# JohannesErnst/WeaSAL

Hardware: AMD Instinct MI355X
Metric: points/sec fwd+bwd KPFCNN on DALES spheres; achieved HBM GB/s on KPConv gather (higher is better)
Workload: dtype f32; 1 GPU; DALES_PseudoLabel KP-FCNN, in_radius=10m, 50k pts/sphere, batch=8, fp32, step = GPU pyramid + fwd + loss + bwd + SGD; contrast_loss term included (trainer_PseudoLabel.py:204-208); pyramid of the next batch overlapped on a second stream; parallelism=dp1, dist_world_size=1, allreduce_bytes=0

## Files before the change

### include/weasal_hip.h

```cpp
#ifndef WEASAL_HIP_H
#define WEASAL_HIP_H

#include <stdint.h>

#ifdef __cplusplus
extern "C" {
#endif

typedef enum {
    WS_OK = 0,
    WS_ERR_INVALID = 1,
    WS_ERR_UNSUPPORTED = 2,
    WS_ERR_HIP = 3,
    WS_ERR_EMPTY = 4,
    WS_ERR_CAPACITY = 5
} ws_status;

enum { WS_INFLUENCE_LINEAR = 0, WS_INFLUENCE_CONSTANT = 1, WS_INFLUENCE_GAUSSIAN = 2 };
enum { WS_AGGREGATION_SUM = 0, WS_AGGREGATION_CLOSEST = 1 };

const char* ws_last_error(void);
int64_t ws_launch_count(void);
const char* ws_version(void);
int ws_device_count(void);
// ... 87 lines not shown
int ws_radius_neighbors_fill(ws_neighbors_ws* ws, int32_t width,
                             int32_t* out_i32, int64_t* out_i64, void* stream);
int ws_radius_neighbors_search(ws_neighbors_ws* ws,
                               const float* queries, int64_t nq, const float* supports, int64_t ns,
                               const int32_t* h_q_lens, const int32_t* h_s_lens, int32_t nb,
                               float radius, int32_t width, int32_t* out_i32, int64_t* out_i64,
                               int32_t* h_max_count, void* stream);
int32_t ws_radius_neighbors_async_cap(int32_t width);
int ws_radius_neighbors_search_async(ws_neighbors_ws* ws,
                                     const float* queries, int64_t nq, const float* supports, int64_t ns,
                                     const int32_t* h_q_lens, const int32_t* h_s_lens, int32_t nb,
                                     float radius, int32_t width, int32_t* out_i32, int64_t* out_i64,
                                     int32_t* d_max_count, void* stream);
#define WS_NB_HIST_MAX 8192
int ws_radius_neighbors_histogram(ws_neighbors_ws* ws,
                                  const float* queries, int64_t nq, const float* supports, int64_t ns,
                                  const int32_t* h_q_lens, const int32_t* h_s_lens, int32_t nb,
                                  float radius, int64_t* hist, int32_t hist_n, void* stream);
int ws_radius_neighbors_nearest_async(ws_neighbors_ws* ws, const float* queries, int64_t nq, const float* supports,
                                      int64_t ns, const int32_t* h_q_lens, const int32_t* h_s_lens, int32_t nb,
                                      float radius, int32_t* out_i32, int64_t* out_i64, int32_t* d_any, void* stream);
int ws_radius_neighbors_order(const ws_neighbors_ws* ws, int32_t* out_order, void* stream);
const int32_t* ws_radius_neighbors_counts(const ws_neighbors_ws* ws);
int ws_radius_neighbors_fill_variant(int32_t cap, int32_t out_i32, int32_t beside, char* out, int32_t out_cap);
int ws_radius_neighbors_last_fills(const ws_neighbors_ws* ws, int32_t* caps, int32_t max, int32_t* n);

#define WS_NN_STATUS_NONFINITE_QUERY 1
int ws_nearest_neighbors(ws_neighbors_ws* ws,
                         const float* queries, int64_t nq, const float* supports, int64_t ns,
                         const int32_t* h_q_lens, const int32_t* h_s_lens, int32_t nb,
                         float cell, int32_t* out_i32, int64_t* out_i64, double* out_d2, int32_t* d_status, void* stream);

int ws_radius_neighbors_set_key_last(ws_neighbors_ws* ws, uint64_t* d_key_last);
int ws_radius_neighbors_reuse_grid(ws_neighbors_ws* ws, int32_t on);
int ws_radius_neighbors_grid_info(const ws_neighbors_ws* ws, int32_t* nb, int64_t* cells, int64_t* ns, int64_t* blob_bytes);
int ws_radius_neighbors_grid_export(const ws_neighbors_ws* ws, void* blob, void* stream);
int ws_kpconv_gather_bwd_x_grid(const float* s_pts, int64_t ns, const void* grid_blob, int32_t nb, int64_t cells,
                                const uint64_t* key_last, float radius, const float* dwf, int32_t ci,
                                const float* kernel_points, int32_t k, const float* deformed_kp, const float* modulations,
                                float extent, int32_t influence, int32_t aggregation, const int32_t* order, float* dx,
                                int32_t* overflow, void* stream);

int ws_kpconv_gather_bwd_x_gated(const float* q_pts, int64_t nq, const float* s_pts, int64_t ns,
                                 const int64_t* inds, int32_t h, const int32_t* t_offsets, const int32_t* t_pairs,
                                 const float* dwf, int32_t ci, const float* kernel_points, int32_t k,
                                 const float* deformed_kp, const float* modulations, float extent,
                                 int32_t influence, int32_t aggregation, const int32_t* order, const float* gate_y,
                                 float gate_slope, float* dx, void* stream);
int ws_kpconv_gather_bwd_x_packed(const float* q_pts, int64_t nq, const float* s_pts, int64_t ns,
                                  const int64_t* inds, int32_t h, const int32_t* t_offsets, const int32_t* t_pairs,
                                  const float* dwf, int32_t ci, const float* kernel_points, int32_t k,
                                  const float* deformed_kp, const float* modulations, float extent,
                                  int32_t influence, int32_t aggregation, const int32_t* order, const float* gate_y,
                                  float gate_slope, float* dx, void* stream);
int ws_kpconv_gather_bwd_x_packed_variant(int64_t nq, int64_t ns, int32_t h, int32_t ci, const void* dwf, const void* dx, int32_t deformed,
                                          int32_t modulated, int32_t influence, int32_t aggregation, int32_t rows_bf16, int32_t ordered,
                                          char* out, int32_t cap);
int ws_kpconv_gather_bwd_x_grid_gated(const float* s_pts, int64_t ns, const void* grid_blob, int32_t nb, int64_t cells,
                                      const uint64_t* key_last, float radius, const float* dwf, int32_t ci,
                                      const float* kernel_points, int32_t k, const float* deformed_kp, const float* modulations,
                                      float extent, int32_t influence, int32_t aggregation, const int32_t* order,
                                      const float* gate_y, float gate_slope, const int64_t* rows, int32_t rows_h, float* dx,
                                      int32_t* overflow, void* stream);

enum { WS_ORDER_REFERENCE = 0, WS_ORDER_FIRST_SEEN = 1 };
typedef struct ws_subsample_ws ws_subsample_ws;
// ... 441 lines not shown
```

### weasal_amd/csrc/neighbors.hip

```cpp
#include "neighbors_kernels.h"
#include "nearest_kernels.h"
#include "ws_dispatch.h"
#include <vector>
#include <algorithm>

namespace {

template <typename T>
struct DevBuf {
    T* p = nullptr;
    size_t cap = 0;
    int ensure(size_t n)
    {
        if (n <= cap) return WS_OK;
        if (p) (void)hipFree(p);
        p = nullptr; cap = 0;
        size_t want = n + n / 4 + 64;
        WS_HIP(hipMalloc((void**)&p, want * sizeof(T)));
        cap = want;
        return WS_OK;
    }
    void release() { if (p) (void)hipFree(p); p = nullptr; cap = 0; }
};

}

struct ws_neighbors_ws {
    DevBuf<CloudGrid> grids;
    DevBuf<float> bbox;
    DevBuf<int32_t> cell_of, cell_start, cursor, counts, scan_scratch, max_count;
    DevBuf<float4> sorted, sorted_alt;
    DevBuf<int32_t> order;
    bool self_query = false;
    const float* queries = nullptr;
    int64_t nq = 0, ns = 0;
    int nb = 0;
    float r2 = 0.f;
    int max_count_host = 0;
    int64_t cells = 0;
    int32_t* max_count_word = nullptr;
    unsigned long long* key_last = nullptr;
    bool reuse_next = false;
    const float* supports = nullptr;
    float radius = 0.f;
    bool auto_cell = false;
    std::vector<int32_t> s_lens;
    std::vector<int32_t> fills;
};

extern "C" {

int ws_neighbors_ws_create(ws_neighbors_ws** ws)
{
    WS_REQUIRE(ws, "NULL argument");
    *ws = new ws_neighbors_ws();
    return WS_OK;
}

void ws_neighbors_ws_destroy(ws_neighbors_ws* ws)
{
    if (!ws) return;
    ws->grids.release(); ws->bbox.release(); ws->cell_of.release(); ws->cell_start.release();
    ws->cursor.release(); ws->counts.release(); ws->scan_scratch.release(); ws->max_count.release();
    ws->sorted.release(); ws->sorted_alt.release(); ws->order.release();
    delete ws;
}

static int nb_prepare(ws_neighbors_ws* ws, const float* queries, int64_t nq, const float* supports, int64_t ns,
                      const int32_t* h_q_lens, const int32_t* h_s_lens, int32_t nb, float radius, hipStream_t st,
                      bool auto_cell = false)
{
    WS_REQUIRE(ws && h_q_lens && h_s_lens, "NULL argument");
    ws->fills.clear();
    WS_REQUIRE(nb >= 1 && nq >= 0 && ns >= 0, "bad sizes nb=%d nq=%lld ns=%lld", nb, (long long)nq, (long long)ns);
// ... 89 lines not shown
    return WS_OK;
}

static int nb_begin(ws_neighbors_ws* ws, const float* queries, int64_t nq, const float* supports, int64_t ns,
                    const int32_t* h_q_lens, const int32_t* h_s_lens, int32_t nb, float radius, hipStream_t st,
                    bool auto_cell = false)
{
    const int rc = nb_prepare(ws, queries, nq, supports, ns, h_q_lens, h_s_lens, nb, radius, st, auto_cell);
    if (rc && ws) ws->nq = 0;
    return rc;
}

int ws_radius_neighbors_plan(ws_neighbors_ws* ws, const float* queries, int64_t nq, const float* supports,
                             int64_t ns, const int32_t* h_q_lens, const int32_t* h_s_lens, int32_t nb,
                             float radius, int32_t* h_max_count, void* stream)
{
    WS_REQUIRE(h_max_count, "NULL argument");
    *h_max_count = 0;
    hipStream_t st = (hipStream_t)stream;
    int rc = nb_begin(ws, queries, nq, supports, ns, h_q_lens, h_s_lens, nb, radius, st);
    if (rc) return rc;
    nb_count_kernel<<<ws_grid(nq, 4), 256, 0, st>>>(queries, nq, ws->grids.p, nb, ws->cell_start.p, ws->sorted.p, ws->r2,
                                                    ws->self_query ? ws->order.p : nullptr, ws->counts.p, ws->max_count_word);
    WS_LAUNCH_CHECK();
    int32_t mc = 0;
    WS_HIP(hipMemcpyAsync(&mc, ws->max_count_word, sizeof(int32_t), hipMemcpyDeviceToHost, st));
    WS_HIP(hipStreamSynchronize(st));
    ws->max_count_host = mc;
    *h_max_count = mc;
    if (mc == 0) return ws_fail(WS_ERR_EMPTY, "Error");
    return WS_OK;
}

struct KeyLastGuard {
    ws_neighbors_ws* ws;
    ~KeyLastGuard() { if (ws) ws->key_last = nullptr; }
};

extern "C" int ws_nb_wide_caps = 1;
constexpr int NB_MAX_BLOCKS = 1024;

enum NbFillKernel { NB_FILL_NONE, NB_FILL_NEAREST, NB_FILL_128, NB_FILL_WIDE, NB_FILL_2048 };
struct NbFillPlan {
    NbFillKernel kernel;
    int slab;
    bool out_i32;
    int max_blocks;
};

static NbFillPlan nb_fill_plan(int cap, bool out_i32, bool beside)
{
    if (cap == 0) return {NB_FILL_NEAREST, 0, out_i32, 256 * 16};
    const int slab = cap <= 128 ? 128 : cap <= 576 ? 576 : cap <= 704 ? 704 : cap <= 1024 ? 1024 : cap <= 2048 ? 2048 : 0;
    const NbFillKernel kernel = !slab ? NB_FILL_NONE : slab == 128 ? NB_FILL_128 : slab == 2048 ? NB_FILL_2048 : NB_FILL_WIDE;
    return {kernel, slab, out_i32, beside ? NB_MAX_BLOCKS : 256 * 16};
}
static int nb_fill_unsupported(int cap)
{
    return ws_fail(WS_ERR_UNSUPPORTED, "max neighbour count %d exceeds the 2048-entry sort slab", cap);
}

static int nb_launch_fill(ws_neighbors_ws* ws, int cap, int32_t width, int32_t* out_i32, int64_t* out_i64,
                          bool with_counts, hipStream_t st, bool beside = false)
{
    const NbFillPlan p = nb_fill_plan(cap, out_i32 != nullptr, beside);
    if (p.kernel == NB_FILL_NONE) return nb_fill_unsupported(cap);
    const int grid = ws_grid(ws->nq, 4, p.max_blocks);
    const int32_t* qo = ws->self_query ? ws->order.p : nullptr;
    int32_t* cn = with_counts ? ws->counts.p : nullptr;
    int32_t* mx = with_counts ? ws->max_count_word : nullptr;
    unsigned long long* kl = ws->key_last;
    const bool called = dispatch([&](auto i32, auto sl) {
        using OT = std::conditional_t<i32.value != 0, int32_t, int64_t>;
        OT* out = i32.value ? (OT*)out_i32 : (OT*)out_i64;
        if constexpr (sl.value == 0)
            nb_nearest_kernel<OT><<<grid, 256, 0, st>>>(ws->queries, ws->nq, ws->grids.p, ws->nb, ws->cell_start.p, ws->sorted.p, ws->r2, ws->ns,
                                                        qo, out, ws->max_count_word);
        else if constexpr (sl.value == 128)
            nb_fill128_kernel<OT><<<grid, 256, 0, st>>>(ws->queries, ws->nq, ws->grids.p, ws->nb, ws->cell_start.p, ws->sorted.p, ws->r2, ws->ns,
                                                        width, qo, out, cn, mx, kl);
        else if constexpr (sl.value == 2048)
            nb_fill_kernel<2048, OT><<<grid, 256, 0, st>>>(ws->queries, ws->nq, ws->grids.p, ws->nb, ws->cell_start.p, ws->sorted.p, ws->r2, ws->ns,
                                                           width, qo, out, cn, mx, kl);
        else
            nb_fill_wide_kernel<OT, sl.value><<<grid, 256, 0, st>>>(ws->queries, ws->nq, ws->grids.p, ws->nb, ws->cell_start.p, ws->sorted.p, ws->r2,
                                                                    ws->ns, width, qo, out, cn, mx, kl);
    }, Flag{p.out_i32}, Pick<0, 128, 576, 704, 1024, 2048>{p.slab});
    if (!called) return ws_no_instantiation("neighbour fill: slab=%d (cap=%d)", p.slab, cap);
    WS_LAUNCH_CHECK();
    ws->fills.push_back(cap);
    return WS_OK;
}

int ws_radius_neighbors_fill_variant(int32_t cap, int32_t out_i32, int32_t beside, char* out, int32_t out_cap)
{
    WS_REQUIRE(out && out_cap > 0 && cap >= 0, "bad argument");
    const NbFillPlan p = nb_fill_plan(cap, out_i32 != 0, beside != 0);
    const char* t = p.out_i32 ? "int32" : "int64";
    switch (p.kernel) {
    case NB_FILL_NONE: return nb_fill_unsupported(cap);
    case NB_FILL_NEAREST: snprintf(out, (size_t)out_cap, "nb_nearest_kernel<%s> grid<=%d", t, p.max_blocks); break;
    case NB_FILL_128: snprintf(out, (size_t)out_cap, "nb_fill128_kernel<%s> grid<=%d", t, p.max_blocks); break;
    case NB_FILL_2048: snprintf(out, (size_t)out_cap, "nb_fill_kernel<2048,%s> grid<=%d", t, p.max_blocks); break;
    case NB_FILL_WIDE: snprintf(out, (size_t)out_cap, "nb_fill_wide_kernel<%s,%d> grid<=%d", t, p.slab, p.max_blocks); break;
    }
    return WS_OK;
}

int ws_radius_neighbors_last_fills(const ws_neighbors_ws* ws, int32_t* caps, int32_t max, int32_t* n)
{
    WS_REQUIRE(ws && n && max >= 0 && (caps || max == 0), "NULL argument");
    *n = (int32_t)ws->fills.size();
    for (int32_t i = 0; i < *n && i < max; ++i) caps[i] = ws->fills[(size_t)i];
    return WS_OK;
}

int ws_radius_neighbors_search(ws_neighbors_ws* ws, const float* queries, int64_t nq, const float* supports,
                               int64_t ns, const int32_t* h_q_lens, const int32_t* h_s_lens, int32_t nb,
                               float radius, int32_t width, int32_t* out_i32, int64_t* out_i64,
                               int32_t* h_max_count, void* stream)
{
    KeyLastGuard guard{ws};
    WS_REQUIRE(h_max_count, "NULL argument");
    WS_REQUIRE((out_i32 != nullptr) != (out_i64 != nullptr), "exactly one of out_i32 / out_i64 must be given");
    WS_REQUIRE(width >= 1, "width must be >= 1");
    *h_max_count = 0;
    hipStream_t st = (hipStream_t)stream;
    int rc = nb_begin(ws, queries, nq, supports, ns, h_q_lens, h_s_lens, nb, radius, st);
    if (rc) return rc;
    int cap = width > 128 ? 1024 : 128;
    for (;;) {
        WS_HIP(hipMemsetAsync(ws->max_count_word, 0, sizeof(int32_t), st));
        if ((rc = nb_launch_fill(ws, cap, width, out_i32, out_i64, true, st))) return rc;
        int32_t mc = 0;
        WS_HIP(hipMemcpyAsync(&mc, ws->max_count_word, sizeof(int32_t), hipMemcpyDeviceToHost, st));
        WS_HIP(hipStreamSynchronize(st));
        ws->max_count_host = mc;
        *h_max_count = mc;
        if (mc == 0) return ws_fail(WS_ERR_EMPTY, "Error");
        if (mc <= cap) return WS_OK;
        cap = mc;
    }
}

int32_t ws_radius_neighbors_async_cap(int32_t width)
{
    if (width <= 128) return 128;
    if (!ws_nb_wide_caps) return 1024;
    const int need = width + width / 4;
    return need <= 576 ? 576 : (need <= 704 ? 704 : 1024);
}

int ws_radius_neighbors_search_async(ws_neighbors_ws* ws, const float* queries, int64_t nq, const float* supports,
                                     int64_t ns, const int32_t* h_q_lens, const int32_t* h_s_lens, int32_t nb,
                                     float radius, int32_t width, int32_t* out_i32, int64_t* out_i64,
                                     int32_t* d_max_count, void* stream)
{
    KeyLastGuard guard{ws};
    WS_REQUIRE(d_max_count, "NULL argument");
    WS_REQUIRE((out_i32 != nullptr) != (out_i64 != nullptr), "exactly one of out_i32 / out_i64 must be given");
    WS_REQUIRE(width >= 1, "width must be >= 1");
    hipStream_t st = (hipStream_t)stream;
    int rc = nb_begin(ws, queries, nq, supports, ns, h_q_lens, h_s_lens, nb, radius, st);
    if (rc) return rc;
    const int cap = ws_radius_neighbors_async_cap(width);
    if ((rc = nb_launch_fill(ws, cap, width, out_i32, out_i64, true, st, true))) return rc;
    WS_HIP(hipMemcpyAsync(d_max_count, ws->max_count_word, sizeof(int32_t), hipMemcpyDeviceToDevice, st));
    ws->max_count_host = cap;
    return WS_OK;
}

int ws_radius_neighbors_histogram(ws_neighbors_ws* ws, const float* queries, int64_t nq, const float* supports,
                                  int64_t ns, const int32_t* h_q_lens, const int32_t* h_s_lens, int32_t nb,
                                  float radius, int64_t* hist, int32_t hist_n, void* stream)
{
    KeyLastGuard guard{ws};
    WS_REQUIRE(hist, "NULL argument");
    WS_REQUIRE(hist_n >= 1, "hist_n must be >= 1");
    if (hist_n > WS_NB_HIST_MAX)
        return ws_fail(WS_ERR_UNSUPPORTED, "hist_n = %d exceeds the %d bins a workgroup keeps in LDS", hist_n, WS_NB_HIST_MAX);
    hipStream_t st = (hipStream_t)stream;
    int rc = nb_begin(ws, queries, nq, supports, ns, h_q_lens, h_s_lens, nb, radius, st);
    if (rc) return rc;
    const int grid = ws_grid(nq, 16, NB_MAX_BLOCKS);
    nb_hist_kernel<<<grid, 256, sizeof(int) * (size_t)hist_n, st>>>(queries, nq, ws->grids.p, nb, ws->cell_start.p, ws->sorted.p, ws->r2,
                                                                     ws->self_query ? ws->order.p : nullptr,
                                                                     reinterpret_cast<unsigned long long*>(hist), hist_n);
    WS_LAUNCH_CHECK();
    return WS_OK;
}

int ws_radius_neighbors_nearest_async(ws_neighbors_ws* ws, const float* queries, int64_t nq, const float* supports,
                                      int64_t ns, const int32_t* h_q_lens, const int32_t* h_s_lens, int32_t nb,
                                      float radius, int32_t* out_i32, int64_t* out_i64, int32_t* d_any, void* stream)
{
    KeyLastGuard guard{ws};
    WS_REQUIRE(d_any, "NULL argument");
    WS_REQUIRE((out_i32 != nullptr) != (out_i64 != nullptr), "exactly one of out_i32 / out_i64 must be given");
    hipStream_t st = (hipStream_t)stream;
    int rc = nb_begin(ws, queries, nq, supports, ns, h_q_lens, h_s_lens, nb, radius, st);
    if (rc) return rc;
    if ((rc = nb_launch_fill(ws, 0, 1, out_i32, out_i64, false, st))) return rc;
    WS_HIP(hipMemcpyAsync(d_any, ws->max_count_word, sizeof(int32_t), hipMemcpyDeviceToDevice, st));
    ws->max_count_host = 1;
    return WS_OK;
}

int ws_radius_neighbors_fill(ws_neighbors_ws* ws, int32_t width, int32_t* out_i32, int64_t* out_i64, void* stream)
{
    KeyLastGuard guard{ws};
    WS_REQUIRE(ws && ws->nq > 0 && ws->max_count_host > 0, "no successful plan to fill from");
    WS_REQUIRE((out_i32 != nullptr) != (out_i64 != nullptr), "exactly one of out_i32 / out_i64 must be given");
    WS_REQUIRE(width >= 1 && width <= ws->max_count_host, "width %d outside [1, max_count=%d]", width, ws->max_count_host);
    ws->fills.clear();
    return nb_launch_fill(ws, ws->max_count_host, width, out_i32, out_i64, false, (hipStream_t)stream);
}

int ws_radius_neighbors_order(const ws_neighbors_ws* ws, int32_t* out_order, void* stream)
{
    WS_REQUIRE(ws && ws->ns > 0 && out_order, "no plan / NULL argument");
    WS_HIP(hipMemcpyAsync(out_order, ws->order.p, sizeof(int32_t) * (size_t)ws->ns, hipMemcpyDeviceToDevice, (hipStream_t)stream));
    return WS_OK;
}

const int32_t* ws_radius_neighbors_counts(const ws_neighbors_ws* ws) { return ws ? ws->counts.p : nullptr; }

int ws_radius_neighbors_reuse_grid(ws_neighbors_ws* ws, int32_t on)
{
    WS_REQUIRE(ws, "NULL argument");
    ws->reuse_next = on != 0;
    return WS_OK;
}

int ws_radius_neighbors_set_key_last(ws_neighbors_ws* ws, uint64_t* d_key_last)
{
    WS_REQUIRE(ws, "NULL argument");
    ws->key_last = reinterpret_cast<unsigned long long*>(d_key_last);
    return WS_OK;
}

int ws_radius_neighbors_grid_info(const ws_neighbors_ws* ws, int32_t* nb, int64_t* cells, int64_t* ns, int64_t* blob_bytes)
{
    WS_REQUIRE(ws && ws->nq > 0 && nb && cells && ns && blob_bytes, "no plan / NULL argument");
    *nb = ws->nb; *cells = ws->cells; *ns = ws->ns;
    *blob_bytes = ws_grid_blob_bytes(ws->nb, ws->cells, ws->ns);
    return WS_OK;
}

int ws_radius_neighbors_grid_export(const ws_neighbors_ws* ws, void* blob, void* stream)
{
    WS_REQUIRE(ws && ws->nq > 0 && blob, "no plan / NULL argument");
    hipStream_t st = (hipStream_t)stream;
    char* base = (char*)blob;
    WS_HIP(hipMemcpyAsync(base, ws->grids.p, sizeof(CloudGrid) * (size_t)ws->nb, hipMemcpyDeviceToDevice, st));
    WS_HIP(hipMemcpyAsync(base + ws_grid_blob_cells_off(ws->nb), ws->cell_start.p, sizeof(int32_t) * (size_t)(ws->cells + 2),
                          hipMemcpyDeviceToDevice, st));
    WS_HIP(hipMemcpyAsync(base + ws_grid_blob_sorted_off(ws->nb, ws->cells), ws->sorted.p, sizeof(float4) * (size_t)ws->ns,
                          hipMemcpyDeviceToDevice, st));
    return WS_OK;
}

int ws_nearest_neighbors(ws_neighbors_ws* ws, const float* queries, int64_t nq, const float* supports, int64_t ns,
                         const int32_t* h_q_lens, const int32_t* h_s_lens, int32_t nb, float cell, int32_t* out_i32,
                         int64_t* out_i64, double* out_d2, int32_t* d_status, void* stream)
{
    KeyLastGuard guard{ws};
    WS_REQUIRE(ws && h_q_lens && h_s_lens, "NULL argument");
    WS_REQUIRE((out_i32 != nullptr) != (out_i64 != nullptr), "exactly one of out_i32 / out_i64 must be given");
    WS_REQUIRE(nb >= 1 && nq >= 0 && ns >= 0, "bad sizes nb=%d nq=%lld ns=%lld", nb, (long long)nq, (long long)ns);
    WS_REQUIRE(ns < (1ll << 30) && nq < (1ll << 31), "point count exceeds int32 range");
    WS_REQUIRE(cell >= 0.f && cell < 3.0e38f, "cell must be finite and >= 0 (0: chosen by the library)");
    int64_t qsum = 0, ssum = 0;
    for (int b = 0; b < nb; ++b) {
        WS_REQUIRE(h_q_lens[b] >= 0 && h_s_lens[b] >= 0, "negative batch length");
        qsum += h_q_lens[b]; ssum += h_s_lens[b];
    }
    WS_REQUIRE(qsum == nq && ssum == ns, "batch lengths do not sum to the point counts (%lld/%lld, %lld/%lld)",
               (long long)qsum, (long long)nq, (long long)ssum, (long long)ns);
    WS_REQUIRE(nq == 0 || queries, "NULL argument");
    WS_REQUIRE(nq == 0 || ns == 0 || supports, "NULL argument");
    if (nq == 0) return WS_OK;
    hipStream_t st = (hipStream_t)stream;
    ws->reuse_next = false;
    if (ns > 0) {
        const int rc = nb_begin(ws, queries, nq, supports, ns, h_q_lens, h_s_lens, nb, cell, st, cell == 0.f);
        if (rc) return rc;
    }
    const int grid = ws_grid(nq, 256);
    dispatch([&](auto i32) {
        using OT = std::conditional_t<i32.value != 0, int32_t, int64_t>;
        OT* out = i32.value ? (OT*)out_i32 : (OT*)out_i64;
        if (ns == 0)
            nn_none_kernel<OT><<<grid, 256, 0, st>>>(nq, ns, out, out_d2);
        else
            nn_exact_kernel<OT><<<grid, 256, 0, st>>>(queries, nq, ws->grids.p, nb, ws->cell_start.p, ws->sorted.p, ns,
                                                      ws->self_query ? ws->order.p : nullptr, out, out_d2, d_status);
    }, Flag{out_i32 != nullptr});
    WS_LAUNCH_CHECK();
    ws->nq = 0;
// ... 7 lines not shown
```

### weasal_amd/csrc/neighbors_kernels.h

```cpp
#pragma once
#include "ws_scan.h"
#include "ws_grid.h"

namespace {

__global__ __launch_bounds__(1024) void nb_bbox_kernel(const float* __restrict__ pts, CloudGrid* __restrict__ grids,
                                                        float* __restrict__ bbox )
{
    __shared__ float red[6][16];
    const CloudGrid g = grids[blockIdx.x];
    float mn[3] = {3.4e38f, 3.4e38f, 3.4e38f}, mx[3] = {-3.4e38f, -3.4e38f, -3.4e38f};
    for (int i = threadIdx.x; i < g.s_len; i += blockDim.x) {
        const float* p = pts + 3 * (int64_t)(g.s_base + i);
#pragma unroll
        for (int d = 0; d < 3; ++d) { mn[d] = fminf(mn[d], p[d]); mx[d] = fmaxf(mx[d], p[d]); }
    }
    const int lane = threadIdx.x & 63, wave = threadIdx.x >> 6;
#pragma unroll
    for (int d = 0; d < 3; ++d) {
#pragma unroll
        for (int o = 32; o > 0; o >>= 1) {
            mn[d] = fminf(mn[d], __shfl_xor(mn[d], o, 64));
            mx[d] = fmaxf(mx[d], __shfl_xor(mx[d], o, 64));
        }
        if (lane == 0) { red[d][wave] = mn[d]; red[3 + d][wave] = mx[d]; }
    }
    __syncthreads();
    if (threadIdx.x < 6) {
        const int d = threadIdx.x;
        float v = red[d][0];
        for (int w = 1; w < (int)(blockDim.x >> 6); ++w) v = d < 3 ? fminf(v, red[d][w]) : fmaxf(v, red[d][w]);
        bbox[blockIdx.x * 6 + d] = v;
    }
}

// ... 219 lines not shown
        if (cnt > 1) {
            for (int k = 2; k <= m; k <<= 1) {
                for (int j = k >> 1; j > 0; j >>= 1) {
                    for (int t = lane; t < (m >> 1); t += 64) {
                        const int i = ((t & ~(j - 1)) << 1) | (t & (j - 1));
                        const int l = i | j;
                        const unsigned long long a = slab[i], bb = slab[l];
                        const bool up = (i & k) == 0;
                        if ((a > bb) == up) { slab[i] = bb; slab[l] = a; }
                    }
                    wave_lds_sync();
                }
            }
        }
        for (int j = lane; j < width; j += 64)
            out[q * width + j] = j < cnt ? (OutT)nb_key_index(slab[j]) : (OutT)ns;
        if (key_last && lane == 0) key_last[q] = cnt > width ? slab[width - 1] : ~0ull;
        wave_lds_sync();
    }
    if (max_count) nb_publish_max(max_count, local_max, lane);
}

template <typename OutT>
__global__ __launch_bounds__(256) void nb_fill128_kernel(const float* __restrict__ queries, int64_t nq,
                                                          const CloudGrid* __restrict__ grids, int nb,
                                                          const int32_t* __restrict__ cell_start,
                                                          const float4* __restrict__ sorted, float r2, int64_t ns,
                                                          int width, const int32_t* __restrict__ qorder, OutT* __restrict__ out,
                                                          int32_t* __restrict__ counts, int32_t* __restrict__ max_count,
                                                          unsigned long long* __restrict__ key_last)
{
    constexpr int CAP = 128;
    __shared__ unsigned long long slab_all[4][CAP + 64];
    const int wave = __builtin_amdgcn_readfirstlane(threadIdx.x >> 6), lane = threadIdx.x & 63;
    unsigned long long* slab = slab_all[wave];
    int local_max = 0;
    int64_t ibeg, iend;
    ws_block_range(nq, ibeg, iend);
    int b = 0;
    CloudGrid g = grids[0];
    for (int64_t it = ibeg + wave; it < iend; it += 4) {
        const int64_t q = qorder ? (int64_t)qorder[it] : it;
        if (q < g.q_base || q >= g.q_base + g.q_len) {
            b = find_cloud_q(grids, nb, q);
            g = grids[b];
        }
        const float qx = queries[3 * q], qy = queries[3 * q + 1], qz = queries[3 * q + 2];
        int cnt = 0;
        auto take = [&](const float4& c, bool active) {
            const float d2 = ref_d2(qx, qy, qz, c);
            const int2 put = slab_compact(active && d2 < r2, CAP, lane, cnt);
            slab[put.x] = nb_key(d2, (unsigned)__float_as_int(c.w));
            cnt = put.y;
        };
        if (g.s_len > 0) {
            grid_walk(g, qx, qy, qz, cell_start, sorted, lane, take);
        }
        if (counts) {
            if (lane == 0) counts[q] = cnt;
            local_max = max(local_max, cnt);
        }
        cnt = min(cnt, CAP);
        wave_lds_sync();
        const unsigned long long a = lane < cnt ? slab[lane] : ~0ull;
        const unsigned long long bkey = lane + 64 < cnt ? slab[lane + 64] : ~0ull;
        __shared__ int hist_all[4][64];
        __shared__ unsigned char member_all[4][128];
        int* hist = hist_all[wave];
        unsigned char* member = member_all[wave];
        hist[lane] = 0;
        wave_lds_sync();
        const float bscale = 64.0f / r2;
        const int ba = min(63, (int)(nb_key_d2(a) * bscale));
        const int bb = min(63, (int)(nb_key_d2(bkey) * bscale));
        int pa = 0, pb = 0;
        if (lane < cnt) pa = atomicAdd(&hist[ba], 1);
        if (lane + 64 < cnt) pb = atomicAdd(&hist[bb], 1);
        wave_lds_sync();
        const int own = hist[lane];
        int incl = own;
#pragma unroll
        for (int o = 1; o < 64; o <<= 1) {
            const int t = __shfl_up(incl, o, 64);
            incl += lane >= o ? t : 0;
        }
        int maxb = own;
#pragma unroll
        for (int o = 32; o > 0; o >>= 1) maxb = max(maxb, __shfl_xor(maxb, o, 64));
        maxb = __builtin_amdgcn_readfirstlane(maxb);
        __shared__ int start_all[4][64];
        int* start = start_all[wave];
        start[lane] = incl - own;
        wave_lds_sync();
        const int sa = start[ba], sb = start[bb];
        const int na = lane < cnt ? hist[ba] : 0, nbk = lane + 64 < cnt ? hist[bb] : 0;
        if (lane < cnt) member[sa + pa] = (unsigned char)lane;
        if (lane + 64 < cnt) member[sb + pb] = (unsigned char)(lane + 64);
        wave_lds_sync();
        int ra = sa, rb = sb;
        for (int t = 0; t < maxb; ++t) {
            const bool oka = t < na, okb = t < nbk;
            const unsigned long long ka = slab[member[oka ? sa + t : 0]];
            const unsigned long long kb = slab[member[okb ? sb + t : 0]];
            ra += (oka && ka < a) ? 1 : 0;
            rb += (okb && kb < bkey) ? 1 : 0;
        }
        OutT* orow = out + q * width;
        if (lane < cnt && ra < width) orow[ra] = (OutT)nb_key_index(a);
        if (lane + 64 < cnt && rb < width) orow[rb] = (OutT)nb_key_index(bkey);
        for (int j = cnt + lane; j < width; j += 64) orow[j] = (OutT)ns;
        if (key_last) {
            if (cnt > width) {
                if (lane < cnt && ra == width - 1) key_last[q] = a;
                if (lane + 64 < cnt && rb == width - 1) key_last[q] = bkey;
            } else if (lane == 0) {
                key_last[q] = ~0ull;
            }
        }
        wave_lds_sync();
    }
    if (max_count) nb_publish_max(max_count, local_max, lane);
}

template <typename OutT>
__global__ __launch_bounds__(256) void nb_nearest_kernel(const float* __restrict__ queries, int64_t nq,
                                                          const CloudGrid* __restrict__ grids, int nb,
                                                          const int32_t* __restrict__ cell_start,
                                                          const float4* __restrict__ sorted, float r2, int64_t ns,
                                                          const int32_t* __restrict__ qorder, OutT* __restrict__ out,
                                                          int32_t* __restrict__ any_hit)
{
    const int wave = __builtin_amdgcn_readfirstlane(threadIdx.x >> 6), lane = threadIdx.x & 63;
    int64_t ibeg, iend;
    ws_block_range(nq, ibeg, iend);
    int b = 0;
    CloudGrid g = grids[0];
    int found_any = 0;
    for (int64_t it = ibeg + wave; it < iend; it += 4) {
        const int64_t q = qorder ? (int64_t)qorder[it] : it;
        if (q < g.q_base || q >= g.q_base + g.q_len) {
            b = find_cloud_q(grids, nb, q);
            g = grids[b];
        }
        const float qx = queries[3 * q], qy = queries[3 * q + 1], qz = queries[3 * q + 2];
        unsigned long long best = ~0ull;
        if (g.s_len > 0) {
            const CellRuns u = grid_cell_runs(g, qx, qy, qz, cell_start);
            float4 c[9];
#pragma unroll
            for (int r = 0; r < 9; ++r) {
                const int p = u.rb[r] + lane;
// ... 194 lines not shown
```

### weasal_amd/csrc/pyramid.hip

```cpp
#include "ws_common.h"
#include "ws_grid.h"
#include <string.h>
#include <algorithm>

namespace {

inline int64_t al256(int64_t b) { return (b + 255) / 256 * 256; }

struct Bump {
    char* base; int64_t cap, used;
    int64_t take(int64_t bytes) { const int64_t o = used; used += al256(bytes > 0 ? bytes : 1); return o; }
};

__global__ __launch_bounds__(256) void pyr_trim_kernel(const int64_t* __restrict__ src, int64_t rows, int w, int mc,
                                                        int64_t* __restrict__ dst)
{
    const int64_t total = rows * (int64_t)mc;
    for (int64_t i = (int64_t)blockIdx.x * 256 + threadIdx.x; i < total; i += (int64_t)gridDim.x * 256)
        dst[i] = src[(i / mc) * w + (i % mc)];
}

template <typename Place>
int pyr_subsample_level(ws_subsample_ws* sws, ws_pyramid_desc* d, int l, const float* pts_l, float* tmp_a, float* tmp_b,
                        Place&& place, const float** next, hipStream_t st)
// ... 127 lines not shown
        if (d->conv_on[l]) {
            if (last_s == pts[l] && last_r == d->r_conv[l]) { if ((rc = ws_radius_neighbors_reuse_grid(nws, 1))) return rc; }
            if (d->want_grids)
                if ((rc = ws_radius_neighbors_set_key_last(nws, (uint64_t*)(A.base + d->off_key_last[l])))) return rc;
            d->cap[3 * l] = ws_radius_neighbors_async_cap(d->limit[l]);
            if ((rc = ws_radius_neighbors_search_async(nws, pts[l], n, pts[l], n, d->lens[l], d->lens[l], nb, d->r_conv[l], d->limit[l],
                                                       nullptr, (int64_t*)(A.base + d->off_neighbors[l]), slots + 3 * l, st)))
                return rc;
            last_s = pts[l]; last_r = d->r_conv[l];
            d->width[3 * l] = d->limit[l];
            if ((rc = ws_radius_neighbors_order(nws, (int32_t*)(A.base + d->off_order[l]), st))) return rc;
            if (d->want_grids) {
                int32_t gnb = 0; int64_t cells = 0, gns = 0, bytes = 0;
                if ((rc = ws_radius_neighbors_grid_info(nws, &gnb, &cells, &gns, &bytes))) return rc;
                WS_REQUIRE(bytes == d->blob_bytes[l] && cells == d->grid_cells[l], "grid export size differs from the planned one");
                if ((rc = ws_radius_neighbors_grid_export(nws, A.base + d->off_blob[l], st))) return rc;
            }
        }
        if (d->pool_on[l]) {
            const int64_t m = d->n[l + 1];
            if (last_s == pts[l] && last_r == d->r_pool[l]) { if ((rc = ws_radius_neighbors_reuse_grid(nws, 1))) return rc; }
            d->cap[3 * l + 1] = ws_radius_neighbors_async_cap(d->limit[l]);
            if ((rc = ws_radius_neighbors_search_async(nws, pts[l + 1], m, pts[l], n, d->lens[l + 1], d->lens[l], nb, d->r_pool[l],
                                                       d->limit[l], nullptr, (int64_t*)(A.base + d->off_pools[l]), slots + 3 * l + 1, st)))
                return rc;
            last_s = pts[l]; last_r = d->r_pool[l];
            d->width[3 * l + 1] = d->limit[l];
            const float r_up = d->r_up[l];
            d->cap[3 * l + 2] = ws_radius_neighbors_async_cap(d->nearest_up ? 1 : d->limit[l + 1]);
            if (d->nearest_up) {
                if ((rc = ws_radius_neighbors_nearest_async(nws, pts[l], n, pts[l + 1], m, d->lens[l], d->lens[l + 1], nb, r_up, nullptr,
                                                            (int64_t*)(A.base + d->off_upsamples[l]), slots + 3 * l + 2, st)))
                    return rc;
            } else if ((rc = ws_radius_neighbors_search_async(nws, pts[l], n, pts[l + 1], m, d->lens[l], d->lens[l + 1], nb, r_up,
                                                              d->limit[l + 1], nullptr, (int64_t*)(A.base + d->off_upsamples[l]),
                                                              slots + 3 * l + 2, st)))
                return rc;
            last_s = pts[l + 1]; last_r = r_up;
            d->width[3 * l + 2] = d->nearest_up ? 1 : d->limit[l + 1];
        }
    }
    for (int l = 0; l < L; ++l)
        WS_HIP(hipMemcpyAsync(A.base + d->off_lens + (int64_t)l * nb * 4, d->lens[l], (size_t)nb * 4, hipMemcpyHostToDevice, st));
    int32_t host_slots[3 * WS_PYRAMID_MAX_LEVELS];
    WS_HIP(hipMemcpyAsync(host_slots, slots, (size_t)(3 * L) * 4, hipMemcpyDeviceToHost, st));
    WS_HIP(hipStreamSynchronize(st));
    for (int l = 0; l < L; ++l)
        for (int k = 0; k < 3; ++k)
            if (d->width[3 * l + k] > 0) d->max_count[3 * l + k] = host_slots[3 * l + k];
    for (int l = 0; l < L; ++l)
        for (int k = 0; k < 3; ++k) {
            const int w = d->width[3 * l + k], mc = d->max_count[3 * l + k];
            if (w <= 0) continue;
            if (mc <= 0 || mc > d->cap[3 * l + k]) continue;
            d->final_width[3 * l + k] = w;
            if (mc < w) {
                const int64_t rows = k == 1 ? d->n[l + 1] : d->n[l];
                int64_t* mat = (int64_t*)(A.base + (k == 0 ? d->off_neighbors[l] : (k == 1 ? d->off_pools[l] : d->off_upsamples[l])));
                pyr_trim_kernel<<<ws_grid(rows * mc, 256), 256, 0, st>>>(mat, rows, w, mc, (int64_t*)d->scratch);
                WS_LAUNCH_CHECK();
                WS_HIP(hipMemcpyAsync(mat, d->scratch, (size_t)(rows * mc) * 8, hipMemcpyDeviceToDevice, st));
                d->final_width[3 * l + k] = mc;
            }
        }
    if (d->want_tables)
        for (int l = 0; l < L; ++l) {
            const int64_t n = d->n[l];
            if (d->off_toffsets[3 * l] >= 0 && d->final_width[3 * l] > 0) {
                if ((rc = ws_transpose_build((const int64_t*)(A.base + d->off_neighbors[l]), n, d->final_width[3 * l], n,
                                             (int32_t*)(A.base + d->off_toffsets[3 * l]), (int32_t*)(A.base + d->off_tpairs[3 * l]),
// ... 66 lines not shown
```

### weasal_amd/csrc/ws_grid.h

```cpp
#pragma once
#include "ws_common.h"

struct CloudGrid {
    float lo[3];
    float inv_cell;
    int nx, ny, nz;
    int cell_base;
    int cell_cap;
    int s_base, s_len;
    int q_base, q_len;
};

#ifdef __HIPCC__
__device__ __forceinline__ int cell_coord(float v, float lo, float inv)
{
#pragma clang fp contract(off)
    const float d = v - lo;
    const float t = floorf(d * inv);
    return (int)fminf(fmaxf(t, -2.0f), 1.0e6f);
}

__device__ __forceinline__ float ref_d2(float qx, float qy, float qz, const float4& c)
{
#pragma clang fp contract(off)
// ... 57 lines not shown
    CellRuns u;
#pragma unroll
    for (int r = 0; r < 9; ++r) {
        const int2 run = grid_cell_run(g, k, r, cell_start);
        u.rb[r] = run.x;
        u.re[r] = run.y;
    }
    return u;
}

template <typename F>
__device__ __forceinline__ void grid_walk(const CloudGrid g, float x, float y, float z, const int32_t* __restrict__ cell_start,
                                          const float4* __restrict__ sorted, int lane, F f)
{
    const CellRuns u = grid_cell_runs(g, x, y, z, cell_start);
    float4 c[9];
#pragma unroll
    for (int r = 0; r < 9; ++r) {
        const int p = u.rb[r] + lane;
        c[r] = sorted[p < u.re[r] ? p : 0];
    }
#pragma unroll
    for (int r = 0; r < 9; ++r) {
        f(c[r], u.rb[r] + lane < u.re[r]);
        for (int p0 = u.rb[r] + 64; p0 < u.re[r]; p0 += 64) {
            const int p = p0 + lane;
            float4 cc = make_float4(0.f, 0.f, 0.f, 0.f);
            if (p < u.re[r]) cc = sorted[p];
            f(cc, p < u.re[r]);
        }
    }
}

__host__ __device__ inline int64_t ws_grid_blob_align(int64_t b) { return (b + 255) / 256 * 256; }
__host__ __device__ inline int64_t ws_grid_blob_cells_off(int nb) { return ws_grid_blob_align((int64_t)nb * (int64_t)sizeof(CloudGrid)); }
__host__ __device__ inline int64_t ws_grid_blob_sorted_off(int nb, int64_t cells)
{
    return ws_grid_blob_cells_off(nb) + ws_grid_blob_align((cells + 2) * (int64_t)sizeof(int32_t));
}
__host__ __device__ inline int64_t ws_grid_blob_bytes(int nb, int64_t cells, int64_t ns)
{
    return ws_grid_blob_sorted_off(nb, cells) + ns * (int64_t)sizeof(float4);
}
#endif
```

### weasal_amd/ops.py

```python
import os

import numpy as np
import torch

from . import _lib
from ._lib import check, current_stream, ptr
from .hints import BatchHints

_timer = None


def set_kernel_timer(timer):
    global _timer
    _timer = timer


def _tbegin(*key):
    return _timer.begin(key) if _timer is not None else None


def _tend(tok):
    if tok is not None:
        _timer.end(tok)

# ... 848 lines not shown
    _need_cuda(queries, supports, status)
    q = _f32c(queries)
    s = _f32c(supports)
    ql, sl = _host_lens(q_lens), _host_lens(s_lens)
    if ql.shape[0] != sl.shape[0]:
        raise RuntimeError("Wrong number of batch elements: different for queries and supports ")
    if dtype not in (torch.int32, torch.int64):
        raise ValueError("dtype must be torch.int32 or torch.int64")
    if status is not None and (status.dtype != torch.int32 or status.numel() != 1):
        raise ValueError("status must be one int32 word on the device")
    with torch.cuda.device(q.device):
        out = torch.empty(q.shape[0], dtype=dtype, device=q.device)
        d2 = torch.empty(q.shape[0], dtype=torch.float64, device=q.device) if return_d2 else None
        o32, o64 = (ptr(out), None) if dtype == torch.int32 else (None, ptr(out))
        check(lib.ws_nearest_neighbors(_ws.neighbors(q.device), ptr(q), q.shape[0], ptr(s), s.shape[0],
                                       C.c_void_p(ql.ctypes.data), C.c_void_p(sl.ctypes.data), ql.shape[0],
                                       float(np.float32(cell)), o32, o64, ptr(d2), ptr(status), current_stream()))
    return (out, d2) if return_d2 else out


def widen_async_slabs(max_count):
    import ctypes as C
    if max_count <= 1024:
        C.c_int.in_dll(_lib.lib(), "ws_nb_wide_caps").value = 0


class DeferredSearches:

    def __init__(self, device, capacity=64):
        self.device = device
        self.slots = torch.zeros(capacity, dtype=torch.int32, device=device)
        self.calls = []

    def add(self, queries, supports, q_lens, s_lens, radius, limit, want_order=False, want_grid=False, reuse_grid=False):
        import ctypes as C
        lib = _lib.lib()
        q, s = _f32c(queries), _f32c(supports)
        ql, sl = _host_lens(q_lens), _host_lens(s_lens)
        if ql.shape[0] != sl.shape[0]:
            raise RuntimeError("Wrong number of batch elements: different for queries and supports ")
        if len(self.calls) >= self.slots.shape[0]:
            raise RuntimeError("DeferredSearches capacity exceeded")
        ws = _ws.neighbors(q.device)
        width = max(1, int(limit))
        cap = int(lib.ws_radius_neighbors_async_cap(width))
        out = torch.empty((q.shape[0], width), dtype=torch.int64, device=q.device)
        slot = len(self.calls)
        grid = None
        with torch.cuda.device(q.device):
            if reuse_grid:
                check(lib.ws_radius_neighbors_reuse_grid(ws, 1))
            if want_grid:
                grid = SearchGrid()
                grid.max_count = 0
                grid.cap = cap
                grid.key_last = torch.empty((q.shape[0],), dtype=torch.int64, device=q.device)
                grid.radius = float(np.float32(radius))
                grid.overflow = torch.zeros((1,), dtype=torch.int32, device=q.device)
                check(lib.ws_radius_neighbors_set_key_last(ws, ptr(grid.key_last)))
            check(lib.ws_radius_neighbors_search_async(
                ws, ptr(q), q.shape[0], ptr(s), s.shape[0], C.c_void_p(ql.ctypes.data), C.c_void_p(sl.ctypes.data),
                ql.shape[0], float(np.float32(radius)), width, None, ptr(out),
                C.c_void_p(self.slots.data_ptr() + 4 * slot), current_stream()))
            order = None
            if want_order:
                order = torch.empty(s.shape[0], dtype=torch.int32, device=q.device)
                check(lib.ws_radius_neighbors_order(ws, ptr(order), current_stream()))
            if want_grid:
                nb, cells, ns_, nbytes = C.c_int32(0), C.c_int64(0), C.c_int64(0), C.c_int64(0)
                check(lib.ws_radius_neighbors_grid_info(ws, C.byref(nb), C.byref(cells), C.byref(ns_), C.byref(nbytes)))
                grid.blob = torch.empty((nbytes.value,), dtype=torch.uint8, device=q.device)
                grid.nb, grid.cells, grid.ns = nb.value, cells.value, ns_.value
                check(lib.ws_radius_neighbors_grid_export(ws, ptr(grid.blob), current_stream()))
        self.calls.append((out, (q, s, ql, sl, radius, width, cap)))
        if want_grid:
            return out, order, grid
        return (out, order) if want_order else out

    def finish(self):
        counts = self.slots[:len(self.calls)].cpu().numpy() if self.calls else []
        self.last_counts = [int(c) for c in counts]
        final = []
        for (out, args), mc in zip(self.calls, counts):
            q, s, ql, sl, radius, width, cap = args
            if mc == 0:
                raise _lib.WeasalHipError("libweasal_hip status 4: Error")
            if mc > cap:
                widen_async_slabs(mc)
                out = radius_neighbors(q, s, ql, sl, radius, limit=width, dtype=torch.int64)
            elif mc < width:
                out = out[:, :int(mc)].contiguous()
            final.append(out)
# ... 683 lines not shown
```

Measured before the change: 32.95 million points/s.

## Walk queries in spatial order and cache grid cell block across queries

The upsample neighbour search now visits queries in a spatially sorted order taken from the conv level. Each wave handles a contiguous chunk of that order instead of a strided one, and keeps the last 3x3 cell-run block plus the first candidate loads, so neighbouring queries reuse them. It also prefetches the next query's coordinates and uses a single-half rank path when there are at most 64 candidates. The aim is fewer redundant cell_start and sorted loads and less LDS ranking work, at the cost of more registers per lane for the cached float4s, which may lower occupancy.

After: 33.23 million points/s (median of 6 runs). About the same (+0.9%).

```diff
diff --git a/include/weasal_hip.h b/include/weasal_hip.h
--- a/include/weasal_hip.h
+++ b/include/weasal_hip.h
@@ -143,6 +143,7 @@
                          float cell, int32_t* out_i32, int64_t* out_i64, double* out_d2, int32_t* d_status, void* stream);
 
 int ws_radius_neighbors_set_key_last(ws_neighbors_ws* ws, uint64_t* d_key_last);
+int ws_radius_neighbors_set_query_order(ws_neighbors_ws* ws, const int32_t* d_order);
 int ws_radius_neighbors_reuse_grid(ws_neighbors_ws* ws, int32_t on);
 int ws_radius_neighbors_grid_info(const ws_neighbors_ws* ws, int32_t* nb, int64_t* cells, int64_t* ns, int64_t* blob_bytes);
 int ws_radius_neighbors_grid_export(const ws_neighbors_ws* ws, void* blob, void* stream);
diff --git a/weasal_amd/csrc/neighbors.hip b/weasal_amd/csrc/neighbors.hip
--- a/weasal_amd/csrc/neighbors.hip
+++ b/weasal_amd/csrc/neighbors.hip
@@ -40,6 +40,7 @@
     int64_t cells = 0;
     int32_t* max_count_word = nullptr;
     unsigned long long* key_last = nullptr;
+    const int32_t* query_order = nullptr;
     bool reuse_next = false;
     const float* supports = nullptr;
     float radius = 0.f;
@@ -195,9 +196,9 @@
     return WS_OK;
 }
 
-struct KeyLastGuard {
+struct OneShotGuard {
     ws_neighbors_ws* ws;
-    ~KeyLastGuard() { if (ws) ws->key_last = nullptr; }
+    ~OneShotGuard() { if (ws) { ws->key_last = nullptr; ws->query_order = nullptr; } }
 };
 
 extern "C" int ws_nb_wide_caps = 1;
@@ -229,7 +230,7 @@
     const NbFillPlan p = nb_fill_plan(cap, out_i32 != nullptr, beside);
     if (p.kernel == NB_FILL_NONE) return nb_fill_unsupported(cap);
     const int grid = ws_grid(ws->nq, 4, p.max_blocks);
-    const int32_t* qo = ws->self_query ? ws->order.p : nullptr;
+    const int32_t* qo = ws->self_query ? ws->order.p : ws->query_order;
     int32_t* cn = with_counts ? ws->counts.p : nullptr;
     int32_t* mx = with_counts ? ws->max_count_word : nullptr;
     unsigned long long* kl = ws->key_last;
@@ -283,7 +284,7 @@
                                float radius, int32_t width, int32_t* out_i32, int64_t* out_i64,
                                int32_t* h_max_count, void* stream)
 {
-    KeyLastGuard guard{ws};
+    OneShotGuard guard{ws};
     WS_REQUIRE(h_max_count, "NULL argument");
     WS_REQUIRE((out_i32 != nullptr) != (out_i64 != nullptr), "exactly one of out_i32 / out_i64 must be given");
     WS_REQUIRE(width >= 1, "width must be >= 1");
@@ -319,7 +320,7 @@
                                      float radius, int32_t width, int32_t* out_i32, int64_t* out_i64,
                                      int32_t* d_max_count, void* stream)
 {
-    KeyLastGuard guard{ws};
+    OneShotGuard guard{ws};
     WS_REQUIRE(d_max_count, "NULL argument");
     WS_REQUIRE((out_i32 != nullptr) != (out_i64 != nullptr), "exactly one of out_i32 / out_i64 must be given");
     WS_REQUIRE(width >= 1, "width must be >= 1");
@@ -337,7 +338,7 @@
                                   int64_t ns, const int32_t* h_q_lens, const int32_t* h_s_lens, int32_t nb,
                                   float radius, int64_t* hist, int32_t hist_n, void* stream)
 {
-    KeyLastGuard guard{ws};
+    OneShotGuard guard{ws};
     WS_REQUIRE(hist, "NULL argument");
     WS_REQUIRE(hist_n >= 1, "hist_n must be >= 1");
     if (hist_n > WS_NB_HIST_MAX)
@@ -357,7 +358,7 @@
                                       int64_t ns, const int32_t* h_q_lens, const int32_t* h_s_lens, int32_t nb,
                                       float radius, int32_t* out_i32, int64_t* out_i64, int32_t* d_any, void* stream)
 {
-    KeyLastGuard guard{ws};
+    OneShotGuard guard{ws};
     WS_REQUIRE(d_any, "NULL argument");
     WS_REQUIRE((out_i32 != nullptr) != (out_i64 != nullptr), "exactly one of out_i32 / out_i64 must be given");
     hipStream_t st = (hipStream_t)stream;
@@ -371,7 +372,7 @@
 
 int ws_radius_neighbors_fill(ws_neighbors_ws* ws, int32_t width, int32_t* out_i32, int64_t* out_i64, void* stream)
 {
-    KeyLastGuard guard{ws};
+    OneShotGuard guard{ws};
     WS_REQUIRE(ws && ws->nq > 0 && ws->max_count_host > 0, "no successful plan to fill from");
     WS_REQUIRE((out_i32 != nullptr) != (out_i64 != nullptr), "exactly one of out_i32 / out_i64 must be given");
     WS_REQUIRE(width >= 1 && width <= ws->max_count_host, "width %d outside [1, max_count=%d]", width, ws->max_count_host);
@@ -399,6 +400,13 @@
 {
     WS_REQUIRE(ws, "NULL argument");
     ws->key_last = reinterpret_cast<unsigned long long*>(d_key_last);
+    return WS_OK;
+}
+
+int ws_radius_neighbors_set_query_order(ws_neighbors_ws* ws, const int32_t* d_order)
+{
+    WS_REQUIRE(ws, "NULL argument");
+    ws->query_order = d_order;
     return WS_OK;
 }
 
@@ -427,7 +435,7 @@
                          const int32_t* h_q_lens, const int32_t* h_s_lens, int32_t nb, float cell, int32_t* out_i32,
                          int64_t* out_i64, double* out_d2, int32_t* d_status, void* stream)
 {
-    KeyLastGuard guard{ws};
+    OneShotGuard guard{ws};
     WS_REQUIRE(ws && h_q_lens && h_s_lens, "NULL argument");
     WS_REQUIRE((out_i32 != nullptr) != (out_i64 != nullptr), "exactly one of out_i32 / out_i64 must be given");
     WS_REQUIRE(nb >= 1 && nq >= 0 && ns >= 0, "bad sizes nb=%d nq=%lld ns=%lld", nb, (long long)nq, (long long)ns);
diff --git a/weasal_amd/csrc/neighbors_kernels.h b/weasal_amd/csrc/neighbors_kernels.h
--- a/weasal_amd/csrc/neighbors_kernels.h
+++ b/weasal_amd/csrc/neighbors_kernels.h
@@ -1,6 +1,7 @@
 #pragma once
 #include "ws_scan.h"
 #include "ws_grid.h"
+#include <type_traits>
 
 namespace {
 
@@ -286,20 +287,38 @@
 {
     constexpr int CAP = 128;
     __shared__ unsigned long long slab_all[4][CAP + 64];
+    __shared__ int hist_all[4][64];
+    __shared__ unsigned char member_all[4][128];
+    __shared__ int start_all[4][64];
     const int wave = __builtin_amdgcn_readfirstlane(threadIdx.x >> 6), lane = threadIdx.x & 63;
     unsigned long long* slab = slab_all[wave];
+    int* hist = hist_all[wave];
+    unsigned char* member = member_all[wave];
+    int* start = start_all[wave];
+    const float bscale = 64.0f / r2;
     int local_max = 0;
     int64_t ibeg, iend;
     ws_block_range(nq, ibeg, iend);
+    const int64_t per = (iend - ibeg + 3) >> 2;
+    const int64_t wbeg = min(ibeg + wave * per, iend), wend = min(wbeg + per, iend);
     int b = 0;
     CloudGrid g = grids[0];
-    for (int64_t it = ibeg + wave; it < iend; it += 4) {
-        const int64_t q = qorder ? (int64_t)qorder[it] : it;
+    CellBlockCache kept = grid_block_cache_none();
+    int64_t qn = 0;
+    float nx = 0.f, ny = 0.f, nz = 0.f;
+    if (wbeg < wend) {
+        qn = qorder ? (int64_t)qorder[wbeg] : wbeg;
+        nx = queries[3 * qn]; ny = queries[3 * qn + 1]; nz = queries[3 * qn + 2];
+    }
+    for (int64_t it = wbeg; it < wend; ++it) {
+        const int64_t q = qn;
+        const float qx = nx, qy = ny, qz = nz;
+        const int64_t itn = it + 1 < wend ? it + 1 : it;
+        qn = qorder ? (int64_t)qorder[itn] : itn;
         if (q < g.q_base || q >= g.q_base + g.q_len) {
             b = find_cloud_q(grids, nb, q);
             g = grids[b];
         }
-        const float qx = queries[3 * q], qy = queries[3 * q + 1], qz = queries[3 * q + 2];
         int cnt = 0;
         auto take = [&](const float4& c, bool active) {
             const float d2 = ref_d2(qx, qy, qz, c);
@@ -308,69 +327,74 @@
             cnt = put.y;
         };
         if (g.s_len > 0) {
-            grid_walk(g, qx, qy, qz, cell_start, sorted, lane, take);
-        }
+            kept = grid_walk_cached(kept, b, g, qx, qy, qz, cell_start, sorted, lane, take);
+        }
+        nx = queries[3 * qn]; ny = queries[3 * qn + 1]; nz = queries[3 * qn + 2];
         if (counts) {
             if (lane == 0) counts[q] = cnt;
             local_max = max(local_max, cnt);
         }
         cnt = min(cnt, CAP);
         wave_lds_sync();
-        const unsigned long long a = lane < cnt ? slab[lane] : ~0ull;
-        const unsigned long long bkey = lane + 64 < cnt ? slab[lane + 64] : ~0ull;
-        __shared__ int hist_all[4][64];
-        __shared__ unsigned char member_all[4][128];
-        int* hist = hist_all[wave];
-        unsigned char* member = member_all[wave];
-        hist[lane] = 0;
-        wave_lds_sync();
-        const float bscale = 64.0f / r2;
-        const int ba = min(63, (int)(nb_key_d2(a) * bscale));
-        const int bb = min(63, (int)(nb_key_d2(bkey) * bscale));
-        int pa = 0, pb = 0;
-        if (lane < cnt) pa = atomicAdd(&hist[ba], 1);
-        if (lane + 64 < cnt) pb = atomicAdd(&hist[bb], 1);
-        wave_lds_sync();
-        const int own = hist[lane];
-        int incl = own;
-#pragma unroll
-        for (int o = 1; o < 64; o <<= 1) {
-            const int t = __shfl_up(incl, o, 64);
-            incl += lane >= o ? t : 0;
-        }
-        int maxb = own;
-#pragma unroll
-        for (int o = 32; o > 0; o >>= 1) maxb = max(maxb, __shfl_xor(maxb, o, 64));
-        maxb = __builtin_amdgcn_readfirstlane(maxb);
-        __shared__ int start_all[4][64];
-        int* start = start_all[wave];
-        start[lane] = incl - own;
-        wave_lds_sync();
-        const int sa = start[ba], sb = start[bb];
-        const int na = lane < cnt ? hist[ba] : 0, nbk = lane + 64 < cnt ? hist[bb] : 0;
-        if (lane < cnt) member[sa + pa] = (unsigned char)lane;
-        if (lane + 64 < cnt) member[sb + pb] = (unsigned char)(lane + 64);
-        wave_lds_sync();
-        int ra = sa, rb = sb;
-        for (int t = 0; t < maxb; ++t) {
-            const bool oka = t < na, okb = t < nbk;
-            const unsigned long long ka = slab[member[oka ? sa + t : 0]];
-            const unsigned long long kb = slab[member[okb ? sb + t : 0]];
-            ra += (oka && ka < a) ? 1 : 0;
-            rb += (okb && kb < bkey) ? 1 : 0;
-        }
-        OutT* orow = out + q * width;
-        if (lane < cnt && ra < width) orow[ra] = (OutT)nb_key_index(a);
-        if (lane + 64 < cnt && rb < width) orow[rb] = (OutT)nb_key_index(bkey);
-        for (int j = cnt + lane; j < width; j += 64) orow[j] = (OutT)ns;
-        if (key_last) {
-            if (cnt > width) {
-                if (lane < cnt && ra == width - 1) key_last[q] = a;
-                if (lane + 64 < cnt && rb == width - 1) key_last[q] = bkey;
-            } else if (lane == 0) {
-                key_last[q] = ~0ull;
-            }
-        }
+        auto rank_and_store = [&](auto two) {
+            constexpr bool TWO = decltype(two)::value;
+            const unsigned long long a = lane < cnt ? slab[lane] : ~0ull;
+            unsigned long long bkey = ~0ull;
+            if constexpr (TWO) bkey = lane + 64 < cnt ? slab[lane + 64] : ~0ull;
+            hist[lane] = 0;
+            wave_lds_sync();
+            const int ba = min(63, (int)(nb_key_d2(a) * bscale));
+            const int bb = min(63, (int)(nb_key_d2(bkey) * bscale));
+            int pa = 0, pb = 0;
+            if (lane < cnt) pa = atomicAdd(&hist[ba], 1);
+            if constexpr (TWO) { if (lane + 64 < cnt) pb = atomicAdd(&hist[bb], 1); }
+            wave_lds_sync();
+            const int own = hist[lane];
+            int incl = own;
+#pragma unroll
+            for (int o = 1; o < 64; o <<= 1) {
+                const int t = __shfl_up(incl, o, 64);
+                incl += lane >= o ? t : 0;
+            }
+            int maxb = own;
+#pragma unroll
+            for (int o = 32; o > 0; o >>= 1) maxb = max(maxb, __shfl_xor(maxb, o, 64));
+            maxb = __builtin_amdgcn_readfirstlane(maxb);
+            start[lane] = incl - own;
+            wave_lds_sync();
+            const int sa = start[ba];
+            const int na = lane < cnt ? hist[ba] : 0;
+            int sb = 0, nbk = 0;
+            if constexpr (TWO) { sb = start[bb]; nbk = lane + 64 < cnt ? hist[bb] : 0; }
+            if (lane < cnt) member[sa + pa] = (unsigned char)lane;
+            if constexpr (TWO) { if (lane + 64 < cnt) member[sb + pb] = (unsigned char)(lane + 64); }
+            wave_lds_sync();
+            int ra = sa, rb = sb;
+            for (int t = 0; t < maxb; ++t) {
+                const bool oka = t < na;
+                const unsigned long long ka = slab[member[oka ? sa + t : 0]];
+                ra += (oka && ka < a) ? 1 : 0;
+                if constexpr (TWO) {
+                    const bool okb = t < nbk;
+                    const unsigned long long kb = slab[member[okb ? sb + t : 0]];
+                    rb += (okb && kb < bkey) ? 1 : 0;
+                }
+            }
+            OutT* orow = out + q * width;
+            if (lane < cnt && ra < width) orow[ra] = (OutT)nb_key_index(a);
+            if constexpr (TWO) { if (lane + 64 < cnt && rb < width) orow[rb] = (OutT)nb_key_index(bkey); }
+            for (int j = cnt + lane; j < width; j += 64) orow[j] = (OutT)ns;
+            if (key_last) {
+                if (cnt > width) {
+                    if (lane < cnt && ra == width - 1) key_last[q] = a;
+                    if constexpr (TWO) { if (lane + 64 < cnt && rb == width - 1) key_last[q] = bkey; }
+                } else if (lane == 0) {
+                    key_last[q] = ~0ull;
+                }
+            }
+        };
+        if (cnt <= 64) rank_and_store(std::false_type{});
+        else rank_and_store(std::true_type{});
         wave_lds_sync();
     }
     if (max_count) nb_publish_max(max_count, local_max, lane);
diff --git a/weasal_amd/csrc/pyramid.hip b/weasal_amd/csrc/pyramid.hip
--- a/weasal_amd/csrc/pyramid.hip
+++ b/weasal_amd/csrc/pyramid.hip
@@ -183,10 +183,14 @@
                 if ((rc = ws_radius_neighbors_nearest_async(nws, pts[l], n, pts[l + 1], m, d->lens[l], d->lens[l + 1], nb, r_up, nullptr,
                                                             (int64_t*)(A.base + d->off_upsamples[l]), slots + 3 * l + 2, st)))
                     return rc;
-            } else if ((rc = ws_radius_neighbors_search_async(nws, pts[l], n, pts[l + 1], m, d->lens[l], d->lens[l + 1], nb, r_up,
-                                                              d->limit[l + 1], nullptr, (int64_t*)(A.base + d->off_upsamples[l]),
-                                                              slots + 3 * l + 2, st)))
-                return rc;
+            } else {
+                if (d->conv_on[l])
+                    if ((rc = ws_radius_neighbors_set_query_order(nws, (const int32_t*)(A.base + d->off_order[l])))) return rc;
+                if ((rc = ws_radius_neighbors_search_async(nws, pts[l], n, pts[l + 1], m, d->lens[l], d->lens[l + 1], nb, r_up,
+                                                           d->limit[l + 1], nullptr, (int64_t*)(A.base + d->off_upsamples[l]),
+                                                           slots + 3 * l + 2, st)))
+                    return rc;
+            }
             last_s = pts[l + 1]; last_r = r_up;
             d->width[3 * l + 2] = d->nearest_up ? 1 : d->limit[l + 1];
         }
diff --git a/weasal_amd/csrc/ws_grid.h b/weasal_amd/csrc/ws_grid.h
--- a/weasal_amd/csrc/ws_grid.h
+++ b/weasal_amd/csrc/ws_grid.h
@@ -113,6 +113,50 @@
     }
 }
 
+struct CellBlockCache { int b; CellBlock k; CellRuns u; float4 c[9]; };
+__device__ __forceinline__ CellBlockCache grid_block_cache_none()
+{
+    CellBlockCache h;
+    h.b = -1;
+    h.k = CellBlock{0, 0, 0, 0};
+#pragma unroll
+    for (int r = 0; r < 9; ++r) { h.u.rb[r] = 0; h.u.re[r] = 0; h.c[r] = make_float4(0.f, 0.f, 0.f, 0.f); }
+    return h;
+}
+template <typename F>
+__device__ __forceinline__ CellBlockCache grid_walk_cached(CellBlockCache h, int b, const CloudGrid g, float x, float y, float z,
+                                                           const int32_t* __restrict__ cell_start,
+                                                           const float4* __restrict__ sorted, int lane, F f)
+{
+    const CellBlock k = grid_cell_block(g, x, y, z);
+    if (b != h.b || k.x0 != h.k.x0 || k.x1 != h.k.x1 || k.cy != h.k.cy || k.cz != h.k.cz) {
+        h.b = b;
+        h.k = k;
+#pragma unroll
+        for (int r = 0; r < 9; ++r) {
+            const int2 run = grid_cell_run(g, k, r, cell_start);
+            h.u.rb[r] = run.x;
+            h.u.re[r] = run.y;
+        }
+#pragma unroll
+        for (int r = 0; r < 9; ++r) {
+            const int p = h.u.rb[r] + lane;
+            h.c[r] = sorted[p < h.u.re[r] ? p : 0];
+        }
+    }
+#pragma unroll
+    for (int r = 0; r < 9; ++r) {
+        f(h.c[r], h.u.rb[r] + lane < h.u.re[r]);
+        for (int p0 = h.u.rb[r] + 64; p0 < h.u.re[r]; p0 += 64) {
+            const int p = p0 + lane;
+            float4 cc = make_float4(0.f, 0.f, 0.f, 0.f);
+            if (p < h.u.re[r]) cc = sorted[p];
+            f(cc, p < h.u.re[r]);
+        }
+    }
+    return h;
+}
+
 __host__ __device__ inline int64_t ws_grid_blob_align(int64_t b) { return (b + 255) / 256 * 256; }
 __host__ __device__ inline int64_t ws_grid_blob_cells_off(int nb) { return ws_grid_blob_align((int64_t)nb * (int64_t)sizeof(CloudGrid)); }
 __host__ __device__ inline int64_t ws_grid_blob_sorted_off(int nb, int64_t cells)
diff --git a/weasal_amd/ops.py b/weasal_amd/ops.py
--- a/weasal_amd/ops.py
+++ b/weasal_amd/ops.py
@@ -904,7 +904,8 @@
         self.slots = torch.zeros(capacity, dtype=torch.int32, device=device)
         self.calls = []
 
-    def add(self, queries, supports, q_lens, s_lens, radius, limit, want_order=False, want_grid=False, reuse_grid=False):
+    def add(self, queries, supports, q_lens, s_lens, radius, limit, want_order=False, want_grid=False, reuse_grid=False,
+            query_order=None):
         import ctypes as C
         lib = _lib.lib()
         q, s = _f32c(queries), _f32c(supports)
@@ -930,6 +931,11 @@
                 grid.radius = float(np.float32(radius))
                 grid.overflow = torch.zeros((1,), dtype=torch.int32, device=q.device)
                 check(lib.ws_radius_neighbors_set_key_last(ws, ptr(grid.key_last)))
+            if query_order is not None:
+                if query_order.dtype != torch.int32 or not query_order.is_contiguous() or query_order.shape != (q.shape[0],) \
+                        or query_order.device != q.device:
+                    raise ValueError("query_order must be a contiguous int32 tensor of one entry per query, on the queries' device")
+                check(lib.ws_radius_neighbors_set_query_order(ws, ptr(query_order)))
             check(lib.ws_radius_neighbors_search_async(
                 ws, ptr(q), q.shape[0], ptr(s), s.shape[0], C.c_void_p(ql.ctypes.data), C.c_void_p(sl.ctypes.data),
                 ql.shape[0], float(np.float32(radius)), width, None, ptr(out),
```
